# Audio-WestlakeU/FN-SSL

Hardware: AMD Instinct MI355X
Metric: TF-frames/sec DP-IPD forward, 4-mic 257-bin x 300-frame (higher is better)
Workload: dtype f32; 1 GPU; BASELINE configs[1]: FN-SSL (online) DP-IPD forward, waveform->STFT->features->3x(full-band BiLSTM + narrow-band LSTM)->head; 32 utterances/GPU x 4 mics ('MM' = 6 pairs) x 257 bins x 300 frames, fp32; frame = one STFT frame of one utterance; stream_chunk_frames=0, utterances_per_gpu=32, global_batch=32, mics=4, pairs_per_utterance=6, frames=300, bins=257, parallelism=dp1 (utterance shards, no collective), chunk_pairs=0

## Files before the change

fn-ssl_amd/csrc/lstm_f32c.h:

```cpp
#pragma once

#include "lstm_static.h"

namespace fnssl_lstm {

constexpr int kF32cWaves = 16;

struct F32ClusterParams {
  unsigned* tags;
  unsigned* status;
  int clusters_per_dir;
  int groups_per_cluster;
  unsigned spin_limit;
  int stall_member;
  int rotate;
  int prio_mode;
};

template <int HH, int NV0, int NS0, int MODE, bool ABLRT = false, int DRIFT = 2, int NW_ = kF32cWaves, int GS = 1>
__global__ void __launch_bounds__(NW_ * 64) lstm_f32c_kernel(const LstmParams p, const F32ClusterParams cp) {
  constexpr int H = HH, NS = H / 16, NW = NW_;
  constexpr int NWS = NW / GS;
  static_assert((GS == 1 || GS == 4) && NW % GS == 0 && (NWS & (NWS - 1)) == 0, "gate split: whole slots, a power of two of them");
  constexpr bool SUM = (MODE & kSum) != 0, SAVE = (MODE & kSave) != 0;
  constexpr bool CAT = (MODE & kHas2) != 0;
  constexpr int QPS = 1 + NV0 + NS0 + NS;
  constexpr int XD = NW_ > 12 ? 4 : 8;
  constexpr bool STRH = H == 256 && GS == 1 && NW_ > 8;
  static_assert((CAT ? NS0 == 1 : !(NV0 && NS0)) && (NV0 == 0 || NV0 % XD == 0) && (H == 128 || H == 256),
                "blocks of src0, or its remainder alone, or blocks of src0 + the remainder quad of src2");
  static_assert(H == 128 || NW_ <= 8 || STRH, "H = 256 with the row of h_{t-1} held: at most two waves per SIMD (register budget)");
  static_assert(!STRH || (NV0 >= XD && (NV0 + NS) % XD == 0), "streamed row: the ring depth divides the block count");
  static_assert(GS == 1 || (!SAVE && !ABLRT), "gate split: inference kernels only");
  extern __shared__ __attribute__((aligned(16))) char smem[];
  const int ABL = ABLRT ? p.ablate : 0;

  const int b = blockIdx.x;
  const int m = (b >> 3) % NS;
  const int cl = ((b >> 3) / NS) * 8 + (b & 7);
  if (cl >= cp.clusters_per_dir * p.ndir) return;
  const int dir = cl / cp.clusters_per_dir;
  const int ck = cl - dir * cp.clusters_per_dir;
  const int g0 = ck * cp.groups_per_cluster;
  const int g1 = g0 + cp.groups_per_cluster < p.ntasks ? g0 + cp.groups_per_cluster : p.ntasks;
  if (__hip_atomic_load(cp.status, __ATOMIC_RELAXED, __HIP_MEMORY_SCOPE_AGENT) != 0) return;
  if (cl == 0 && m == cp.stall_member) return;

  const int lane = threadIdx.x & 63;
  const int n = lane & 15, g = lane >> 4;
  const int w = __builtin_amdgcn_readfirstlane((int)(threadIdx.x >> 6));
  const int ws = GS == 1 ? w : (w >> 2);
  const int gate = GS == 1 ? 0 : (w & 3);
  const bool rev = dir == 1;
  const unsigned vlane = lane * 16;

  {
    const v4f* src = reinterpret_cast<const v4f*>(reinterpret_cast<const char*>(p.wpack[dir]) + (size_t)(m * QPS) * 4096);
    v4f* dst = reinterpret_cast<v4f*>(smem);
    for (int i = threadIdx.x; i < QPS * 4 * 64; i += NW * 64) dst[i] = src[i];
  }
  char* const xch = smem + QPS * 4096;
  unsigned* const xcnt = reinterpret_cast<unsigned*>(xch + NWS * 2 * 4 * 1024);
  if (GS > 1 && threadIdx.x < NWS) xcnt[threadIdx.x] = 0;
  __syncthreads();
  const char* const lds_rd = smem + lane * 16;
  auto rec = [&](int q, int j) { return *reinterpret_cast<const v4f*>(lds_rd + (q * 4 + j) * 1024); };
  auto rec1 = [&](int q, int j) { return *reinterpret_cast<const float*>(lds_rd + (q * 4 + j) * 1024 + 4 * gate); };

  const unsigned st0 = (unsigned)(p.src0.st * 4), sto = (unsigned)(p.out_st * 4), stk = SUM ? (unsigned)(p.skip.st * 4) : 0u;
  const unsigned st2 = CAT ? (unsigned)(p.src2.st * 4) : 0u;
  const unsigned cy = (unsigned)p.carry;
  unsigned* const tag_cl = cp.tags + (size_t)cl * cp.groups_per_cluster * NS;
  const v4f zero4 = v4f{0.f, 0.f, 0.f, 0.f};

  unsigned pub_val = 0;
  unsigned* pub_tag = nullptr;
  auto pub_flush = [&]() {
    if (pub_tag) {
      asm volatile("s_waitcnt vmcnt(0)" ::: "memory");
      if (lane == 0) __hip_atomic_store(pub_tag, pub_val, __ATOMIC_RELAXED, __HIP_MEMORY_SCOPE_AGENT);
      pub_tag = nullptr;
    }
  };

  struct Grp {
    unsigned vo0, voo, vok, voo2, vo2 = 0;
    bool valid;
    int task, step;
  };
  auto locate = [&](int task, int qo0, int qi0, Grp& gr, rsrc_t& rx0, rsrc_t& ro, rsrc_t& rsk, rsrc_t& ro2, rsrc_t& rx2) {
    const int q0 = task * 16;
    gr.valid = q0 + n < p.nseq;
    const int d = q0 + n < p.nseq ? n : p.nseq - 1 - q0;
    const bool crossed = qi0 + d >= p.q_inner;
    auto one = [&](const float* base, long long so, long long si, int extra, unsigned& voff) {
      const long long delta = (long long)d * si + (crossed ? so - (long long)p.q_inner * si : 0ll);
      voff = (unsigned)(delta * 4) + (unsigned)(extra * 4);
      return make_rsrc(base + ((long long)qo0 * so + (long long)qi0 * si));
    };
    rx0 = one(p.src0.p, p.src0.so, p.src0.si, (NS0 && !CAT) ? g : 4 * g, gr.vo0);
    if constexpr (CAT) rx2 = one(p.src2.p, p.src2.so, p.src2.si, g, gr.vo2);
    ro = one(p.out, p.out_so, p.out_si, dir * H + 4 * g, gr.voo);
    gr.vok = gr.voo2 = 0;
    rsk = SUM ? one(p.skip.p, p.skip.so, p.skip.si, dir * H + 4 * g, gr.vok) : rx0;
    ro2 = SUM ? one(p.out_sum, p.out_so, p.out_si, dir * H + 4 * g, gr.voo2) : ro;
  };
  auto tt_of = [&](int step) { return (unsigned)(rev ? p.nsteps - 1 - step : step); };
  auto rc_of = [&](int task) {
    return make_rsrc(cell_record<NS>(p.cscratch, p.ntasks, dir, task));
  };

  if (g0 + ws >= g1) return;
  unsigned long long clk0 = 0, rt0 = 0;
  if (ABLRT && (ABL & 512)) {
    clk0 = __builtin_amdgcn_s_memtime();
    rt0 = __builtin_amdgcn_s_memrealtime();
  }
  bool dead = false;
  auto bounded_wait = [&](auto ready, auto reload, int sleep, unsigned code) {
    for (unsigned spins = 0; !ready(); ++spins) {
      if (GS > 1) __builtin_amdgcn_s_sleep(1); else if (sleep == 8) __builtin_amdgcn_s_sleep(8); else __builtin_amdgcn_s_sleep(16);
      reload();
      const bool out = spins > cp.spin_limit;
      if (out || (spins & 63) == 63) {
        if (out) {
          if (lane == 0) __hip_atomic_store(cp.status, code | (unsigned)(cl & 0xffff), __ATOMIC_RELAXED, __HIP_MEMORY_SCOPE_AGENT);
          return false;
        }
        if (__hip_atomic_load(cp.status, __ATOMIC_RELAXED, __HIP_MEMORY_SCOPE_AGENT) != 0) return false;
      }
    }
    return true;
  };
  const int NGR = g1 - g0;
  const bool rot = cp.rotate && NGR >= 2 * NWS;
  const int FULL = rot ? (NGR / NWS) * NWS : NGR, LEFT = NGR - FULL;
  const bool single = GS == 1 && g0 + ws + NWS >= g1;
  Grp cur, nxt;
  rsrc_t rx0, ro, rsk, ro2, rx2, nrx0, nro, nrsk, nro2, nrx2;
  v4f xr[XD];
  float xs0 = 0.f;
  v4f cprev = zero4, skipv = zero4;
  unsigned tagv = 0, tagd = 0;
  auto request = [&](const Grp& gr, rsrc_t qx0, rsrc_t qsk, bool with_c, bool with_x = true) {
    const unsigned tt = tt_of(gr.step);
    if (!(ABL & 8)) {
      if constexpr (NV0 > 0) if (with_x) static_for<XD>([&](auto v) { xr[v.value] = bld4(qx0, gr.vo0, tt * st0 + 64 * v.value); });
      if constexpr (NS0 > 0 && !CAT) xs0 = bld1(qx0, gr.vo0, tt * st0);
    }
    if (SUM && !(ABL & 64)) skipv = bld4(qsk, gr.vok, tt * stk + 64 * m);
    if (gr.step > 0 || cy) {
      if (gr.step > 0 && !(ABL & 256))
        tagv = __hip_atomic_load(tag_cl + (size_t)(gr.task - g0) * NS + (lane & (NS - 1)), __ATOMIC_RELAXED, __HIP_MEMORY_SCOPE_AGENT);
      if (GS == 1 && with_c && !(ABL & 64)) cprev = bld4_l2(rc_of(gr.task), vlane, m * 1024);
    }
    if (DRIFT > 0 && !(ABL & 256) && gr.task - DRIFT * NWS >= g0)
      tagd = __hip_atomic_load(tag_cl + (size_t)(gr.task - DRIFT * NWS - g0) * NS + (lane & (NS - 1)), __ATOMIC_RELAXED, __HIP_MEMORY_SCOPE_AGENT);
  };
  cur.task = g0 + ws;
  cur.step = 0;
  unsigned iter = 0;
  const int qo_first = (cur.task * 16) / p.q_inner, qi_first = cur.task * 16 - qo_first * p.q_inner;
  int qo0 = qo_first, qi0 = qi_first;
  locate(cur.task, qo0, qi0, cur, rx0, ro, rsk, ro2, rx2);
  request(cur, rx0, rsk, true);
  if constexpr (CAT) xs0 = bld1(rx2, cur.vo2, tt_of(0) * st2);

  for (;;) {
    const int step = cur.step, task = cur.task;
    const unsigned tt = tt_of(step);
    const unsigned o0 = tt * st0, oo = (tt + cy) * sto;
    const unsigned op = (rev ? tt + 1 : tt - 1 + cy) * sto;
    const rsrc_t rc = rc_of(task);
    unsigned* const tag_g = tag_cl + (size_t)(task - g0) * NS;
    if (single && (step > 0 || cy) && !(ABL & 64)) cprev = bld4_l2(rc, vlane, m * 1024);
    const bool late_c = GS > 1 || task >= g0 + FULL;
    v4f cprev_cur = (step > 0 || cy) ? cprev : zero4;
    const v4f skip_cur = skipv;

    v4f hold[STRH ? 1 : NS];
    auto fetch_h = [&]() {
      if (DRIFT > 0 && !(ABL & 4) && !dead && task - DRIFT * NWS >= g0) {
        unsigned* const tag_d = tag_cl + (size_t)(task - DRIFT * NWS - g0) * NS;
        dead = !bounded_wait([&]() { return __builtin_amdgcn_ballot_w64(tagd < (unsigned)step + 1) == 0; },
                             [&]() { tagd = __hip_atomic_load(tag_d + (lane & (NS - 1)), __ATOMIC_RELAXED, __HIP_MEMORY_SCOPE_AGENT); }, 8, 0x40000u);
      }
      if ((step > 0 || cy) && !(ABL & 16)) {
        if (step > 0 && !(ABL & 4) && !dead)
          dead = !bounded_wait([&]() { return __builtin_amdgcn_ballot_w64(tagv < (unsigned)step) == 0; },
                               [&]() { tagv = __hip_atomic_load(tag_g + (lane & (NS - 1)), __ATOMIC_RELAXED, __HIP_MEMORY_SCOPE_AGENT); }, 16, 0x30000u);
        if (late_c && !(ABL & 64)) cprev_cur = bld4_l2(rc, vlane, m * 1024);
        if constexpr (!STRH) {
#pragma unroll
          for (int s = 0; s < NS; ++s) hold[s] = bld4_l2(ro, cur.voo, op + 64 * s);
        }
      } else if constexpr (!STRH) {
#pragma unroll
        for (int s = 0; s < NS; ++s) hold[s] = (ABL & 16) ? cprev : zero4;
      }
    };
    const bool hrow = step > 0 || cy;
    auto hblock = [&](int j) { return hrow ? bld4_l2(ro, cur.voo, op + 64 * j) : zero4; };

    if (cp.prio_mode == 2) __builtin_amdgcn_s_setprio(2);
    v4f acc[4];
    v4f ra[4];
    v4f acc1 = zero4;
    float rb[4] = {0.f, 0.f, 0.f, 0.f};
    if constexpr (GS == 1) {
      acc[0] = rec(0, 0);
      acc[1] = rec(0, 1);
      acc[2] = rec(0, 2);
      acc[3] = rec(0, 3);
      static_for<4>([&](auto j) { ra[j.value] = rec(1, j.value); });
    } else {
      acc1 = rec(0, gate);
      static_for<4>([&](auto j) { rb[j.value] = rec1(1, j.value); });
    }
    auto quad = [&](auto qc, float b0, float b1, float b2, float b3) {
      constexpr int Q = decltype(qc)::value;
      if constexpr (GS > 1) {
        acc1 = __builtin_amdgcn_mfma_f32_16x16x4f32(rb[0], b0, acc1, 0, 0, 0);
        if constexpr (Q + 1 < QPS) rb[0] = rec1(Q + 1, 0);
        acc1 = __builtin_amdgcn_mfma_f32_16x16x4f32(rb[1], b1, acc1, 0, 0, 0);
        if constexpr (Q + 1 < QPS) rb[1] = rec1(Q + 1, 1);
        acc1 = __builtin_amdgcn_mfma_f32_16x16x4f32(rb[2], b2, acc1, 0, 0, 0);
        if constexpr (Q + 1 < QPS) rb[2] = rec1(Q + 1, 2);
        acc1 = __builtin_amdgcn_mfma_f32_16x16x4f32(rb[3], b3, acc1, 0, 0, 0);
        if constexpr (Q + 1 < QPS) rb[3] = rec1(Q + 1, 3);
        return;
      }
      MFMA4(acc, ra[0], b0);
      __builtin_amdgcn_sched_barrier(0);
      if constexpr (Q + 1 < QPS) if (!(ABL & 128)) ra[0] = rec(Q + 1, 0);
      __builtin_amdgcn_sched_barrier(0);
// ... 3 lines not shown
      __builtin_amdgcn_sched_barrier(0);
      MFMA4(acc, ra[2], b2);
      __builtin_amdgcn_sched_barrier(0);
      if constexpr (Q + 1 < QPS) if (!(ABL & 128)) ra[2] = rec(Q + 1, 2);
      __builtin_amdgcn_sched_barrier(0);
      MFMA4(acc, ra[3], b3);
      __builtin_amdgcn_sched_barrier(0);
      if constexpr (Q + 1 < QPS) if (!(ABL & 128)) ra[3] = rec(Q + 1, 3);
      __builtin_amdgcn_sched_barrier(0);
    };
    auto quad1 = [&](auto qc, float b0) {
      constexpr int Q = decltype(qc)::value;
      if constexpr (GS > 1) {
        acc1 = __builtin_amdgcn_mfma_f32_16x16x4f32(rb[0], b0, acc1, 0, 0, 0);
        if constexpr (Q + 1 < QPS) static_for<4>([&](auto j) { rb[j.value] = rec1(Q + 1, j.value); });
        return;
      }
      MFMA4(acc, ra[0], b0);
      if constexpr (Q + 1 < QPS) static_for<4>([&](auto j) { ra[j.value] = rec(Q + 1, j.value); });
    };
    if constexpr (NV0 > 0) {
      static_for<NV0>([&](auto v) {
        constexpr int V = decltype(v)::value;
        if constexpr (STRH) {
          if constexpr (V == NV0 / 2) pub_flush();
          if constexpr (V == NV0 - XD) fetch_h();
        } else if constexpr (V == NV0 / 2) {
          pub_flush();
          fetch_h();
        }
        const v4f xb = xr[V % XD];
        quad(ic<1 + V>{}, xb.x, xb.y, xb.z, xb.w);
        if constexpr (V + XD < NV0) {
          if (!(ABL & 8)) xr[V % XD] = bld4(rx0, cur.vo0, o0 + 64 * (V + XD));
        } else if constexpr (STRH) {
          xr[V % XD] = hblock(V + XD - NV0);
        }
      });
      if constexpr (NS0 > 0) quad1(ic<1 + NV0>{}, xs0);
    } else {
      pub_flush();
      fetch_h();
      quad1(ic<1>{}, xs0);
    }
    bool seq_next = false;
    if (task < g0 + FULL && task + NWS < g0 + FULL) {
      nxt.task = task + NWS;
      nxt.step = step;
      seq_next = true;
    } else {
      const int j = (ws - step) & (NWS - 1);
      if (task < g0 + FULL && j < LEFT) {
        nxt.task = g0 + FULL + j;
        nxt.step = step;
      } else {
        nxt.task = g0 + ws;
        nxt.step = step + 1;
      }
    }
    const bool more = nxt.step < p.nsteps;
    if (more) {
      if (ABL & 1) {
        nxt.vo0 = cur.vo0; nxt.voo = cur.voo; nxt.vok = cur.vok; nxt.voo2 = cur.voo2; nxt.valid = cur.valid;
        nrx0 = rx0; nro = ro; nrsk = rsk; nro2 = ro2;
        if constexpr (CAT) {
          nxt.vo2 = cur.vo2;
          nrx2 = rx2;
        }
      } else {
        if (seq_next) {
          qi0 += 16 * NWS;
          while (qi0 >= p.q_inner) {
            qi0 -= p.q_inner;
            ++qo0;
          }
        } else if (nxt.step == step) {
          qo0 = (nxt.task * 16) / p.q_inner;
          qi0 = nxt.task * 16 - qo0 * p.q_inner;
        } else {
          qo0 = qo_first;
          qi0 = qi_first;
        }
        locate(nxt.task, qo0, qi0, nxt, nrx0, nro, nrsk, nro2, nrx2);
      }
      request(nxt, nrx0, nrsk, !single && nxt.task < g0 + FULL, !STRH);
      if constexpr (CAT) xs0 = bld1(nrx2, nxt.vo2, tt_of(nxt.step) * st2);
    }
    static_for<NS>([&](auto sp) {
      constexpr int SP = decltype(sp)::value;
      if constexpr (STRH) {
        constexpr int B = NV0 + SP, B2 = B + XD;
        const v4f hb = xr[B % XD];
        quad(ic<1 + NV0 + NS0 + SP>{}, hb.x, hb.y, hb.z, hb.w);
        if constexpr (B2 < NV0 + NS) {
          xr[B % XD] = hblock(B2 - NV0);
        } else {
          if (more) xr[B % XD] = bld4(nrx0, nxt.vo0, tt_of(nxt.step) * st0 + 64 * (B2 - NV0 - NS));
        }
      } else {
        quad(ic<1 + NV0 + NS0 + SP>{}, hold[SP].x, hold[SP].y, hold[SP].z, hold[SP].w);
      }
    });

    if (cp.prio_mode == 2) __builtin_amdgcn_s_setprio(0);
    if (dead) break;
    v4f cn, hn;
    if (ABL & 2) {
      cn = acc[1] + cprev_cur + acc[0];
      hn = acc[3] + acc[2];
    } else {
      v4f ig, fg, gg, og;
      if constexpr (GS == 1) {
        ig = sigmoid4(acc[0]);
        fg = sigmoid4(acc[1]);
        gg = tanh4(acc[2]);
        og = sigmoid4(acc[3]);
      } else {
        const v4f act = gate == 2 ? tanh4(acc1) : sigmoid4(acc1);
        v4f* const xb = reinterpret_cast<v4f*>(xch + (size_t)((ws * 2 + (int)(iter & 1u)) * 4) * 1024);
        xb[gate * 64 + lane] = act;
        asm volatile("s_waitcnt lgkmcnt(0)" ::: "memory");
        if (lane == 0) __hip_atomic_fetch_add(xcnt + ws, 1u, __ATOMIC_RELAXED, __HIP_MEMORY_SCOPE_WORKGROUP);
        const unsigned want = 4u * (iter + 1u);
        for (unsigned spins = 0;; ++spins) {
          if (__hip_atomic_load(xcnt + ws, __ATOMIC_RELAXED, __HIP_MEMORY_SCOPE_WORKGROUP) >= want) break;
          if (dead || ((spins & 63u) == 63u && __hip_atomic_load(cp.status, __ATOMIC_RELAXED, __HIP_MEMORY_SCOPE_AGENT) != 0u) ||
              spins > cp.spin_limit) {
            dead = true;
            break;
          }
          __builtin_amdgcn_s_sleep(1);
        }
        asm volatile("" ::: "memory");
        ig = xb[lane];
        fg = xb[64 + lane];
        gg = xb[128 + lane];
        og = xb[192 + lane];
        ++iter;
      }
      cn = cell4(fg, cprev_cur, ig, gg);
      hn = mul_rn4(og, tanh4(cn));
      if constexpr (SAVE) {
        const rsrc_t rres = make_rsrc(reinterpret_cast<const char*>(p.reserve) +
                                      ((size_t)dir * p.ntasks + task) * p.nsteps * (size_t)(NS * kReserveRecs * 1024));
        const unsigned rb = (tt * NS + m) * (kReserveRecs * 1024);
        bst4(ig, rres, vlane, rb);
        bst4(fg, rres, vlane, rb + 1024);
        bst4(gg, rres, vlane, rb + 2048);
        bst4(og, rres, vlane, rb + 3072);
        bst4(cn, rres, vlane, rb + 4096);
      }
    }
    asm("" : "+v"(hn.x), "+v"(hn.y), "+v"(hn.z), "+v"(hn.w));
    if (ABL & 32) asm volatile("" ::"v"(cn), "v"(hn));
    const bool storer = GS == 1 || gate == 0;
    if (storer && !(ABL & 32)) bst4(cn, rc, vlane, m * 1024);
    if (storer && cur.valid && !(ABL & 32)) {
      __builtin_amdgcn_raw_buffer_store_b128(__builtin_bit_cast(v4u, hn), ro, cur.voo, oo + 64 * m, 16);
      if (SUM) bst4(add_rn4(hn, skip_cur), ro2, cur.voo2, oo + 64 * m);
    }
    pub_val = __builtin_amdgcn_readfirstlane((unsigned)step + 1);
    pub_tag = ((ABL & 256) || !storer) ? nullptr : tag_g + m;
    if (GS > 1 || single) pub_flush();
    if (!more || dead) break;
    cur = nxt;
    rx0 = nrx0;
    ro = nro;
    rsk = nrsk;
    ro2 = nro2;
    if constexpr (CAT) rx2 = nrx2;
  }
  pub_flush();
  asm volatile("s_waitcnt vmcnt(0)" ::: "memory");
  if (ABLRT && (ABL & 512) && (w == 0 || w == 15) && lane == 0) {
    const unsigned long long c1 = __builtin_amdgcn_s_memtime(), r1 = __builtin_amdgcn_s_memrealtime();
    printf("f32c blk %d wave %d start %llu end %llu cycles %llu MHz %.1f\n", b, w, rt0, r1, c1 - clk0,
           (double)(c1 - clk0) / (double)(r1 - rt0) * 100.0);
  }
}

template <int HH, int NV0, int NS0, int MODE, bool ABLRT = false, int DRIFT = 2, int NW_ = kF32cWaves, int GS = 1>
int launch_f32c_k(const LstmParams& p, const F32ClusterParams& cp, const LaunchCtx& lc) {
  constexpr int NS = HH / 16;
  constexpr int QPS = 1 + NV0 + NS0 + NS;
  const size_t lds = (size_t)QPS * 4096 + (GS > 1 ? (size_t)(NW_ / GS) * 8192 + 64 : 0);
  static_assert(QPS * 4096 + (GS > 1 ? (NW_ / GS) * 8192 + 64 : 0) <= 160 * 1024, "LDS");
  const int ncl = cp.clusters_per_dir * p.ndir;
  const int nwg = 8 * NS * ((ncl + 7) / 8);
  return enqueue(lc, Kernel{lstm_f32c_kernel<HH, NV0, NS0, MODE, ABLRT, DRIFT, NW_, GS>, NW_ * 64, lds, "lstm_f32c_kernel", true}, nwg, p, cp);
}

}
```

fn-ssl_amd/csrc/lstm_f32c.hip:

```cpp
#include <cstdlib>

#include "lstm_f32c.h"
#include "tuning.h"

namespace fnssl_lstm {

constexpr int kF32cWavesH256 = 16;
constexpr int kF32cWavesH256Split = 8;

static bool f32c_uniform(const LstmParams& p, int mode) {
  auto even = [&](long long so, long long si) { return si >= 0 && so == (long long)p.q_inner * si; };
  return even(p.src0.so, p.src0.si) && even(p.out_so, p.out_si) && (!(mode & kSum) || even(p.skip.so, p.skip.si)) &&
         (!(mode & kHas2) || even(p.src2.so, p.src2.si));
}

bool f32c_handles(const LstmParams& p, int H, int mode) {
  if (fnssl::tune(FNSSL_TUNE_NO_F32_CLUSTER)) return false;
  if ((H != 128 && H != 256) || p.ablate) return false;
  if (H == 128) {
    if (p.c2 != 0 || p.carry) return false;
    if (p.reserve && mode != 0) return false;
    if (!(p.c0 == 256 && (mode == kSum || mode == 0)) && !(p.c0 == 4 && mode == 0 && !fnssl::tune(FNSSL_TUNE_NO_F32C_B1))) return false;
  } else {
    if (p.ndir != 1 || p.c0 != 256 || fnssl::tune(FNSSL_TUNE_NO_F32_SMALL)) return false;
    const bool plain = p.c2 == 0 && (mode == 0 || mode == kSum), cat = p.c2 == 4 && (mode == kHas2 || mode == (kHas2 | kSum));
    if (!plain && !cat) return false;
    if (p.reserve && ((mode & kSum) || p.carry)) return false;
  }
  auto grows = [&](long long so, long long si) { return si >= 0 && so >= (long long)(p.q_inner - 1) * si; };
  if (!f32c_uniform(p, mode) &&
      (p.q_inner < 16 || !grows(p.src0.so, p.src0.si) || !grows(p.out_so, p.out_si) ||
       ((mode & kSum) && !grows(p.skip.so, p.skip.si)) || ((mode & kHas2) && !grows(p.src2.so, p.src2.si))))
    return false;
  const int ncu = cluster_cus();
  if (ncu < (H / 16) * p.ndir) return false;
  const long long groups = (long long)p.ntasks * p.ndir;
  if (const int mg = fnssl::tune(FNSSL_TUNE_F32C_MIN_GROUPS, 1, 1 << 30)) {
    if (groups < mg) return false;
  }
  if (p.reserve) {
    if (fnssl::tune(FNSSL_TUNE_TRAIN_NO_F32_CLUSTER)) return false;
    return true;
  }
  if (H == 256) {
    const long long full = 12LL * ncu, rounds = (groups + full - 1) / full;
    return groups < full || groups * 100 < rounds * full * 97;
  }
  return !fnssl::tune(FNSSL_TUNE_NO_F32_SMALL) || groups >= 12LL * ncu;
}

template <int NW_, int GS>
static int launch_f32c_h256(const LstmParams& p, const F32ClusterParams& cp, int mode, const LaunchCtx& lc) {
  if (mode == (kHas2 | kSum)) return launch_f32c_k<256, 16, 1, kHas2 | kSum, false, 2, NW_, GS>(p, cp, lc);
  if (mode == kHas2) return launch_f32c_k<256, 16, 1, kHas2, false, 2, NW_, GS>(p, cp, lc);
  if (mode == kSum) return launch_f32c_k<256, 16, 0, kSum, false, 2, NW_, GS>(p, cp, lc);
  return launch_f32c_k<256, 16, 0, 0, false, 2, NW_, GS>(p, cp, lc);
}

int forward_f32c(LstmParams p, int H, int mode, size_t cluster_bytes, const LaunchCtx& lc) {
  if (f32c_uniform(p, mode)) p.q_inner = p.nseq;
  const int ncu = cluster_cus();
  const int members = H / 16;
  F32ClusterParams cp;
  cp.clusters_per_dir = (ncu / members) / p.ndir;
  cp.groups_per_cluster = (p.ntasks + cp.clusters_per_dir - 1) / cp.clusters_per_dir;
  cp.status = reinterpret_cast<unsigned*>(p.cluster_ws);
  cp.tags = reinterpret_cast<unsigned*>(p.cluster_ws + 256);
  cp.spin_limit = cluster_spin_limit();
  cp.stall_member = cluster_test_stall();
  cp.rotate = !fnssl::tune(FNSSL_TUNE_F32C_NO_ROTATE);
  cp.prio_mode = fnssl::tune(FNSSL_TUNE_F32C_PRIO, 9, 9) ? 0 : 2;
  const size_t tag_bytes = (size_t)p.ndir * cp.clusters_per_dir * cp.groups_per_cluster * members * sizeof(unsigned);
  FNSSL_REQUIRE(256 + tag_bytes <= cluster_bytes, "lstm_forward: the cluster kernel's tags exceed the workspace's cluster area");
  if (!lc.dry) FNSSL_HIP(hipMemsetAsync(p.cluster_ws, 0, 256 + tag_bytes, lc.st));
  const int gs_knob = fnssl::tune(FNSSL_TUNE_F32C_GATE_SPLIT, 1, 4);
  const bool gsplit = gs_knob ? gs_knob == 4 : cp.groups_per_cluster <= 1;
  if (H == 256) {
    constexpr int W = kF32cWavesH256;
    if (p.reserve)
      return p.c2 == 4 ? launch_f32c_k<256, 16, 1, kHas2 | kSave, false, 2, W>(p, cp, lc) : launch_f32c_k<256, 16, 0, kSave, false, 2, W>(p, cp, lc);
    if (gsplit) return launch_f32c_h256<kF32cWavesH256Split, 4>(p, cp, mode, lc);
    if (cp.groups_per_cluster <= kF32cWavesH256Split) return launch_f32c_h256<kF32cWavesH256Split, 1>(p, cp, mode, lc);
    return launch_f32c_h256<W, 1>(p, cp, mode, lc);
  }
  if (gsplit && !p.reserve) {
    if (p.c0 == 4) return launch_f32c_k<128, 0, 1, 0, false, 2, kF32cWaves, 4>(p, cp, lc);
    if (mode == kSum) return launch_f32c_k<128, 16, 0, kSum, false, 2, kF32cWaves, 4>(p, cp, lc);
    return launch_f32c_k<128, 16, 0, 0, false, 2, kF32cWaves, 4>(p, cp, lc);
  }
#ifdef FNSSL_BUILD_ABLATE
  if (const int abl = env_int("FNSSL_F32C_ABL", 1, 1023)) {
    p.ablate = abl;
    if (mode == kSum) return launch_f32c_k<128, 16, 0, kSum, true>(p, cp, lc);
    if (p.c0 == 4) return launch_f32c_k<128, 0, 1, 0, true>(p, cp, lc);
  }
  p.ablate = 0;
#endif
  if (p.reserve) return p.c0 == 4 ? launch_f32c_k<128, 0, 1, kSave>(p, cp, lc) : launch_f32c_k<128, 16, 0, kSave>(p, cp, lc);
  if (p.c0 == 4) return launch_f32c_k<128, 0, 1, 0>(p, cp, lc);
  if (mode == kSum) return launch_f32c_k<128, 16, 0, kSum>(p, cp, lc);
  return launch_f32c_k<128, 16, 0, 0>(p, cp, lc);
}

}
```

fn-ssl_amd/csrc/runtime.hip:

```cpp
#include <atomic>
#include <cstring>
#include <map>
#include <mutex>
#include <string>
#include <vector>

#include "common.h"
#include "tuning.h"
#include "lstm_host.h"

namespace fnssl {

int device_cus() {
  static std::mutex mu;
  static int cache[64] = {0};
  int dev = 0;
  if (hipGetDevice(&dev) != hipSuccess || dev < 0 || dev >= 64) return 256;
  std::lock_guard<std::mutex> lk(mu);
  if (cache[dev] == 0) {
    int n = 0;
    if (hipDeviceGetAttribute(&n, hipDeviceAttributeMultiprocessorCount, dev) != hipSuccess || n <= 0) n = 256;
    cache[dev] = n;
  }
  return cache[dev];
// ... 21 lines not shown
    "LSTM_CHQ",
    "NO_F32_CLUSTER",
    "NO_F32C_B1",
    "TRAIN_NO_F32_CLUSTER",
    "F32C_NO_ROTATE",
    "F32C_PRIO",
    "NO_CLUSTER",
    "NO_CLUSTER_B1",
    "NO_CLUSTER_H128",
    "CLUSTER_SPREAD",
    "BF16P_DRAIN",
    "BF16W_SOLO",
    "BWD_NO_CLUSTER",
    "BWD_CLUSTER_MIN_GROUPS",
    "BWD_CLUSTER_NO_ROTATE",
    "BWDC_NO_PREFETCH",
    "BWDC_NO_TOKEN",
    "BWDC_WAVES16",
    "FWD_RING",
    "BWD_RING",
    "TRAIN_SPLIT",
    "TRAIN_NO_STATIC",
    "NO_FWD2",
    "NO_BWD2",
    "SN_SCALAR",
    "STFT_PER_FRAME",
    "CLUSTER_SPIN_LIMIT",
    "CLUSTER_TEST_STALL",
    "RESERVED_CUS",
    "NO_F32_SMALL",
    "F32C_MIN_GROUPS",
    "F32C_GATE_SPLIT",
    "CLUSTER_FULL_TILES",
    "NO_STATIC4"};
constexpr int kTuneNamed = (int)(sizeof(kTuneNames) / sizeof(kTuneNames[0]));
static_assert(kTuneNamed <= FNSSL_TUNE_COUNT, "more knob names than slots");
static_assert(kTuneNamed == FNSSL_TUNE_NO_STATIC4 + 1, "knob names out of step with include/fnssl.h");
}

const fnssl_tuning& tuning() {
  if (g_call_tuning) return *g_call_tuning;
  const unsigned v = g_tuning_version.load(std::memory_order_acquire);
  if (v != g_thread_version) {
    std::lock_guard<std::mutex> lk(g_tuning_mu);
    g_thread_tuning = g_default_tuning;
    g_thread_version = g_tuning_version.load(std::memory_order_relaxed);
  }
  return g_thread_tuning;
}

TuningScope::TuningScope(const fnssl_tuning* t) : prev_(g_call_tuning), active_(false) {
  if (t && t->struct_bytes == sizeof(fnssl_tuning)) {
    g_call_tuning = t;
    active_ = true;
  }
}
TuningScope::~TuningScope() {
  if (active_) g_call_tuning = prev_;
}

void set_error(const char* fmt, ...) {
  va_list ap;
  va_start(ap, fmt);
  vsnprintf(g_err, sizeof(g_err), fmt, ap);
  va_end(ap);
}

namespace {
struct Rec {
  const char* name;
// ... 215 lines not shown
```

fn-ssl_amd/fnssl/_lib.py:

```python
from __future__ import annotations

import ctypes as C
import os

import torch

_HERE = os.path.dirname(os.path.abspath(__file__))
LIB_PATH = os.path.join(os.path.dirname(_HERE), "csrc", "libfnssl_hip.so")
LIB_PATH = os.environ.get("FNSSL_LIB_PATH", LIB_PATH)

ABI_VERSION = 19
CH_MODE = {"M": 0, "MM": 1}
STREAM_MODE = {"pair": 0, "array": 1}
LSTM_FAMILY = {1: "generic", 2: "static", 3: "static2 (retired)", 4: "split", 5: "split_static", 6: "f32_cluster",
               7: "static3", 8: "bf16", 9: "bf16_solo", 10: "bf16_pair", 11: "bf16_cluster", 12: "train", 13: "bwd", 14: "bwd_cluster",
               15: "static4"}

SYMBOLS = [
    "fnssl_abi_version", "fnssl_last_error", "fnssl_tuning_set", "fnssl_tuning_get", "fnssl_tuning_name", "fnssl_occupy_cus", "fnssl_num_frames", "fnssl_num_pairs", "fnssl_stft",
    "fnssl_num_frames_ex", "fnssl_stft_ex", "fnssl_array_frontend",
    "fnssl_forgetting_coefs", "fnssl_pair_features", "fnssl_nchw_to_seq", "fnssl_lstm_packed_floats",
    "fnssl_lstm_pack", "fnssl_lstm_workspace_bytes", "fnssl_lstm_workspace_bytes_ex", "fnssl_lstm_plan_rounds", "fnssl_lstm_plan", "fnssl_lstm_forward", "fnssl_lstm_cluster_status", "fnssl_head", "fnssl_linear",
    "fnssl_ipd2doa", "fnssl_doa_peaks", "fnssl_dpipd_targets", "fnssl_conv3x3_packed_floats", "fnssl_conv3x3_pack", "fnssl_conv3x3_causal",
    "fnssl_avgpool_time", "fnssl_array_features", "fnssl_conv3x3_packed_floats_bf16", "fnssl_conv3x3_pack_bf16",
# ... 350 lines not shown
    for name in ("fnssl_sn_fconv_backward_workspace_bytes", "fnssl_sn_full_backward_workspace_bytes"):
        getattr(lib, name).argtypes = [i, i, i]
        getattr(lib, name).restype = sz
    lib.fnssl_sn_fconv_backward.argtypes = [PV, i, i, i, C.POINTER(SnFconvW), i, i, vp, ll, ll, ll, vp, ll, ll, ll,
                                            C.POINTER(SnFconvGrads), vp, sz, vp]
    lib.fnssl_sn_full_backward.argtypes = [PV, i, i, i, C.POINTER(SnFullW), i, vp, ll, ll, ll, vp, ll, ll, ll,
                                           C.POINTER(SnFullGrads), vp, sz, vp]
    lib.fnssl_sn_head.argtypes = [PV, i, i, i, vp, vp, vp, vp, vp, vp]
    lib.fnssl_sn_encoder_backward_workspace_bytes.argtypes = [i, i, i, i]
    lib.fnssl_sn_encoder_backward_workspace_bytes.restype = sz
    lib.fnssl_sn_encoder_backward.argtypes = [vp, ll, ll, ll, ll, i, i, i, i, vp, vp, ll, ll, ll, vp, vp, vp, ll, ll, ll, ll,
                                              vp, sz, vp]
    lib.fnssl_sn_head_backward_workspace_bytes.argtypes = [i, i, i]
    lib.fnssl_sn_head_backward_workspace_bytes.restype = sz
    lib.fnssl_sn_head_backward.argtypes = [PV, i, i, i, vp, vp, vp, vp, vp, ll, ll, ll, C.POINTER(SnHeadGrads), vp, sz, vp]
    lib.fnssl_sn_forward_workspace_bytes.argtypes = [i, i, i]
    lib.fnssl_sn_forward_workspace_bytes.restype = sz
    lib.fnssl_sn_state_floats.argtypes = [C.POINTER(SnNet), i, i]
    lib.fnssl_sn_state_floats.restype = sz
    lib.fnssl_sn_forward.argtypes = [C.POINTER(SnNet), vp, ll, ll, ll, ll, i, i, i, vp, i, vp, vp, sz, vp]
    lib.fnssl_sn_state_rows.argtypes = [C.POINTER(SnNet), i, i, vp, i, vp, C.POINTER(C.c_int), C.POINTER(C.c_ubyte), i, vp]
    lib.fnssl_timing_enable.argtypes = [i]
    lib.fnssl_timing_select.argtypes = [C.c_char_p]
    lib.fnssl_timing_collect.argtypes = [i, vp, vp, vp, vp]
    if lib.fnssl_abi_version() != ABI_VERSION:
        raise RuntimeError("fnssl: ABI version mismatch (library %d, binding %d)"
                           % (lib.fnssl_abi_version(), ABI_VERSION))
    _lib = lib
    refresh_tuning()
    return lib


_tune_index = None
_PRESENCE = {"NO_F32_CLUSTER", "NO_F32C_B1", "TRAIN_NO_F32_CLUSTER", "F32C_NO_ROTATE", "NO_CLUSTER", "NO_CLUSTER_B1",
             "NO_CLUSTER_H128", "CLUSTER_SPREAD", "BF16W_SOLO", "SN_SCALAR", "STFT_PER_FRAME"}
_ENV_ALIAS = {"LSTM_NO_STATIC": "FNSSL_LSTM_NO_STATIC"}


def tuning_names():
    global _tune_index
    if _tune_index is None:
        lib = _lib
        if lib is None:
            raise RuntimeError("fnssl: load() first")
        idx, k = {}, 0
        while True:
            n = lib.fnssl_tuning_name(k)
            if n is None:
                break
            idx[n.decode()] = k
            k += 1
        _tune_index = idx
    return _tune_index


def tuning_from_env(environ=None) -> Tuning:
    environ = os.environ if environ is None else environ
    t = Tuning()
    t.struct_bytes = C.sizeof(Tuning)
    for name, k in tuning_names().items():
        v = environ.get(_ENV_ALIAS.get(name, "FNSSL_" + name))
        if v is None:
            continue
        try:
            iv = int(v)
        except ValueError:
            iv = 1
# ... 55 lines not shown
```

include/fnssl.h:

```cpp
#ifndef FNSSL_H_
#define FNSSL_H_

#include <stddef.h>

#ifdef __cplusplus
extern "C" {
#endif

#define FNSSL_ABI_VERSION 19

#define FNSSL_OK 0
#define FNSSL_E_INVALID (-1)
#define FNSSL_E_HIP (-2)
#define FNSSL_E_WORKSPACE (-3)

#define FNSSL_CH_MODE_M 0
#define FNSSL_CH_MODE_MM 1

#define FNSSL_WIN_LEN 512
#define FNSSL_HOP 256
#define FNSSL_NBIN 257
#define FNSSL_NF 256
#define FNSSL_SEG_FRAMES 12

// ... 13 lines not shown
#define FNSSL_TUNE_NO_F32_CLUSTER 9
#define FNSSL_TUNE_NO_F32C_B1 10
#define FNSSL_TUNE_TRAIN_NO_F32_CLUSTER 11
#define FNSSL_TUNE_F32C_NO_ROTATE 12
#define FNSSL_TUNE_F32C_PRIO 13
#define FNSSL_TUNE_NO_CLUSTER 14
#define FNSSL_TUNE_NO_CLUSTER_B1 15
#define FNSSL_TUNE_NO_CLUSTER_H128 16
#define FNSSL_TUNE_CLUSTER_SPREAD 17
#define FNSSL_TUNE_BF16P_DRAIN 18
#define FNSSL_TUNE_BF16W_SOLO 19
#define FNSSL_TUNE_BWD_NO_CLUSTER 20
#define FNSSL_TUNE_BWD_CLUSTER_MIN_GROUPS 21
#define FNSSL_TUNE_BWD_CLUSTER_NO_ROTATE 22
#define FNSSL_TUNE_BWDC_NO_PREFETCH 23
#define FNSSL_TUNE_BWDC_NO_TOKEN 24
#define FNSSL_TUNE_BWDC_WAVES16 25
#define FNSSL_TUNE_FWD_RING 26
#define FNSSL_TUNE_BWD_RING 27
#define FNSSL_TUNE_TRAIN_SPLIT 28
#define FNSSL_TUNE_TRAIN_NO_STATIC 29
#define FNSSL_TUNE_NO_FWD2 30
#define FNSSL_TUNE_NO_BWD2 31
#define FNSSL_TUNE_SN_SCALAR 32
#define FNSSL_TUNE_STFT_PER_FRAME 33
#define FNSSL_TUNE_CLUSTER_SPIN_LIMIT 34
#define FNSSL_TUNE_CLUSTER_TEST_STALL 35
#define FNSSL_TUNE_RESERVED_CUS 36
#define FNSSL_TUNE_NO_F32_SMALL 37
#define FNSSL_TUNE_F32C_MIN_GROUPS 38
#define FNSSL_TUNE_F32C_GATE_SPLIT 39
#define FNSSL_TUNE_CLUSTER_FULL_TILES 40
#define FNSSL_TUNE_NO_STATIC4 41
#define FNSSL_TUNE_COUNT 48

typedef struct fnssl_tuning {
  unsigned struct_bytes;
  int knob[FNSSL_TUNE_COUNT];
} fnssl_tuning;

int fnssl_tuning_set(const fnssl_tuning* t);
int fnssl_tuning_get(fnssl_tuning* t);
const char* fnssl_tuning_name(int index);

int fnssl_occupy_cus(int nblocks, int lds_bytes, unsigned* stop, int max_ms, void* stream);


int fnssl_num_frames(int ns);

int fnssl_num_pairs(int nch, int ch_mode);

int fnssl_stft(const float* sig, int nb, int ns, int nch,
               long long sb, long long sn, long long sc,
               float* spec, float* magsum, void* stream);

int fnssl_num_frames_ex(int ns, int hop, int center);
int fnssl_stft_ex(const float* sig, int nb, int ns, int nch,
                  long long sb, long long sn, long long sc, int hop, int center,
                  float* spec, float* magsum, void* stream);

int fnssl_forgetting_coefs(int nt, int sample_length, float* a, float* b);

int fnssl_pair_features(const float* spec, const float* magsum,
                        const float* coef_a, const float* coef_b,
                        int nb, int nch, int nt, int ch_mode, float eps,
                        float* mu, float* x, int layout, void* stream);
// ... 529 lines not shown
```

Measured before the change: 17120 frames/s.

## Map f32 cluster LSTM task groups onto 2-D sequence tiles for H=128

Adds a tiled mapping for the H=128 f32 cluster LSTM kernel. Each 16-sequence task group becomes an a-by-b tile over the outer/inner sequence axes rather than 16 consecutive sequences, so per-lane offsets are fixed and only a scalar group offset changes between groups. Cell state is addressed per cluster base, and buffer resources are built once. This aims to cut per-group address recomputation and resource rebuilding, and lets strided layouts that previously fell back use the cluster kernel. The cost is more template instances, a new eligibility check, and 32-bit offset limits that the check must respect.

Result: no change. 17180 frames/s (median of 5 runs) (+0.4%).

```diff
diff --git a/fn-ssl_amd/csrc/lstm_f32c.h b/fn-ssl_amd/csrc/lstm_f32c.h
--- a/fn-ssl_amd/csrc/lstm_f32c.h
+++ b/fn-ssl_amd/csrc/lstm_f32c.h
@@ -1,5 +1,6 @@
 #pragma once
 
+#include "lstm_group_tile.h"
 #include "lstm_static.h"
 
 namespace fnssl_lstm {
@@ -17,7 +18,7 @@
   int prio_mode;
 };
 
-template <int HH, int NV0, int NS0, int MODE, bool ABLRT = false, int DRIFT = 2, int NW_ = kF32cWaves, int GS = 1>
+template <int HH, int NV0, int NS0, int MODE, bool ABLRT = false, int DRIFT = 2, int NW_ = kF32cWaves, int GS = 1, bool TILED = false>
 __global__ void __launch_bounds__(NW_ * 64) lstm_f32c_kernel(const LstmParams p, const F32ClusterParams cp) {
   constexpr int H = HH, NS = H / 16, NW = NW_;
   constexpr int NWS = NW / GS;
@@ -32,6 +33,7 @@
   static_assert(H == 128 || NW_ <= 8 || STRH, "H = 256 with the row of h_{t-1} held: at most two waves per SIMD (register budget)");
   static_assert(!STRH || (NV0 >= XD && (NV0 + NS) % XD == 0), "streamed row: the ring depth divides the block count");
   static_assert(GS == 1 || (!SAVE && !ABLRT), "gate split: inference kernels only");
+  static_assert(!TILED || (H == 128 && !SAVE && !CAT && !ABLRT && (!SUM || NV0 > 0)), "tiled groups: the H = 128 inference kernels");
   extern __shared__ __attribute__((aligned(16))) char smem[];
   const int ABL = ABLRT ? p.ablate : 0;
 
@@ -85,10 +87,31 @@
 
   struct Grp {
     unsigned vo0, voo, vok, voo2, vo2 = 0;
+    unsigned s0 = 0, so = 0;
     bool valid;
     int task, step;
   };
+  const GroupTile gt = group_tile(p.q_inner);
+  int qo_base = 0, qi_base = 0;
+  if constexpr (TILED) tile_of_task(g0 + ws, p.q_inner, gt, qo_base, qi_base);
+  const unsigned so4x = tile_stride32(p.src0.so), si4x = tile_stride32(p.src0.si), so4o = tile_stride32(p.out_so), si4o = tile_stride32(p.out_si);
+  const unsigned tvo0 = TILED ? tile_lane_offset32(n, gt, so4x, si4x) + (unsigned)(((NS0 && !CAT) ? g : 4 * g) * 4) : 0u;
+  const unsigned tvoo = TILED ? tile_lane_offset32(n, gt, so4o, si4o) + (unsigned)(4 * g * 4) : 0u;
+  const unsigned sdir = (unsigned)(dir * H * 4);
+  auto V0 = [&](const Grp& gr) { if constexpr (TILED) return tvo0; else return gr.vo0; };
+  auto VO = [&](const Grp& gr) { if constexpr (TILED) return tvoo; else return gr.voo; };
+  auto VK = [&](const Grp& gr) { if constexpr (TILED) return tvo0; else return gr.vok; };
+  auto VO2 = [&](const Grp& gr) { if constexpr (TILED) return tvoo; else return gr.voo2; };
+  auto S0 = [&](const Grp& gr) { if constexpr (TILED) return gr.s0; else return 0u; };
+  auto SO = [&](const Grp& gr) { if constexpr (TILED) return gr.so; else return 0u; };
+  auto SK = [&](const Grp& gr) { if constexpr (TILED) return gr.s0 + sdir; else return 0u; };
   auto locate = [&](int task, int qo0, int qi0, Grp& gr, rsrc_t& rx0, rsrc_t& ro, rsrc_t& rsk, rsrc_t& ro2, rsrc_t& rx2) {
+    if constexpr (TILED) {
+      gr.s0 = tile_group_offset32(qo0, qi0, qo_base, so4x, si4x);
+      gr.so = tile_group_offset32(qo0, qi0, qo_base, so4o, si4o) + sdir;
+      gr.valid = true;
+      return;
+    }
     const int q0 = task * 16;
     gr.valid = q0 + n < p.nseq;
     const int d = q0 + n < p.nseq ? n : p.nseq - 1 - q0;
@@ -107,8 +130,9 @@
   };
   auto tt_of = [&](int step) { return (unsigned)(rev ? p.nsteps - 1 - step : step); };
   auto rc_of = [&](int task) {
-    return make_rsrc(cell_record<NS>(p.cscratch, p.ntasks, dir, task));
-  };
+    return make_rsrc(cell_record<NS>(p.cscratch, p.ntasks, dir, TILED ? g0 : task));
+  };
+  auto cs_of = [&](int task) { return (TILED ? (unsigned)(task - g0) * (unsigned)(NS * 1024) : 0u) + (unsigned)(m * 1024); };
 
   if (g0 + ws >= g1) return;
   unsigned long long clk0 = 0, rt0 = 0;
@@ -145,14 +169,14 @@
   auto request = [&](const Grp& gr, rsrc_t qx0, rsrc_t qsk, bool with_c, bool with_x = true) {
     const unsigned tt = tt_of(gr.step);
     if (!(ABL & 8)) {
-      if constexpr (NV0 > 0) if (with_x) static_for<XD>([&](auto v) { xr[v.value] = bld4(qx0, gr.vo0, tt * st0 + 64 * v.value); });
-      if constexpr (NS0 > 0 && !CAT) xs0 = bld1(qx0, gr.vo0, tt * st0);
-    }
-    if (SUM && !(ABL & 64)) skipv = bld4(qsk, gr.vok, tt * stk + 64 * m);
+      if constexpr (NV0 > 0) if (with_x) static_for<XD>([&](auto v) { xr[v.value] = bld4(qx0, V0(gr), S0(gr) + tt * st0 + 64 * v.value); });
+      if constexpr (NS0 > 0 && !CAT) xs0 = bld1(qx0, V0(gr), S0(gr) + tt * st0);
+    }
+    if (SUM && !(ABL & 64)) skipv = bld4(qsk, VK(gr), SK(gr) + tt * stk + 64 * m);
     if (gr.step > 0 || cy) {
       if (gr.step > 0 && !(ABL & 256))
         tagv = __hip_atomic_load(tag_cl + (size_t)(gr.task - g0) * NS + (lane & (NS - 1)), __ATOMIC_RELAXED, __HIP_MEMORY_SCOPE_AGENT);
-      if (GS == 1 && with_c && !(ABL & 64)) cprev = bld4_l2(rc_of(gr.task), vlane, m * 1024);
+      if (GS == 1 && with_c && !(ABL & 64)) cprev = bld4_l2(rc_of(gr.task), vlane, cs_of(gr.task));
     }
     if (DRIFT > 0 && !(ABL & 256) && gr.task - DRIFT * NWS >= g0)
       tagd = __hip_atomic_load(tag_cl + (size_t)(gr.task - DRIFT * NWS - g0) * NS + (lane & (NS - 1)), __ATOMIC_RELAXED, __HIP_MEMORY_SCOPE_AGENT);
@@ -160,7 +184,16 @@
   cur.task = g0 + ws;
   cur.step = 0;
   unsigned iter = 0;
-  const int qo_first = (cur.task * 16) / p.q_inner, qi_first = cur.task * 16 - qo_first * p.q_inner;
+  int qo_first = (cur.task * 16) / p.q_inner, qi_first = cur.task * 16 - qo_first * p.q_inner;
+  if constexpr (TILED) {
+    qo_first = qo_base;
+    qi_first = qi_base;
+    const long long base = (long long)qo_base;
+    rx0 = nrx0 = make_rsrc(p.src0.p + base * p.src0.so);
+    ro = nro = make_rsrc(p.out + base * p.out_so);
+    rsk = nrsk = SUM ? make_rsrc(p.skip.p + base * p.skip.so) : rx0;
+    ro2 = nro2 = SUM ? make_rsrc(p.out_sum + base * p.out_so) : ro;
+  }
   int qo0 = qo_first, qi0 = qi_first;
   locate(cur.task, qo0, qi0, cur, rx0, ro, rsk, ro2, rx2);
   request(cur, rx0, rsk, true);
@@ -169,11 +202,11 @@
   for (;;) {
     const int step = cur.step, task = cur.task;
     const unsigned tt = tt_of(step);
-    const unsigned o0 = tt * st0, oo = (tt + cy) * sto;
-    const unsigned op = (rev ? tt + 1 : tt - 1 + cy) * sto;
+    const unsigned o0 = S0(cur) + tt * st0, oo = SO(cur) + (tt + cy) * sto;
+    const unsigned op = SO(cur) + (rev ? tt + 1 : tt - 1 + cy) * sto;
     const rsrc_t rc = rc_of(task);
     unsigned* const tag_g = tag_cl + (size_t)(task - g0) * NS;
-    if (single && (step > 0 || cy) && !(ABL & 64)) cprev = bld4_l2(rc, vlane, m * 1024);
+    if (single && (step > 0 || cy) && !(ABL & 64)) cprev = bld4_l2(rc, vlane, cs_of(task));
     const bool late_c = GS > 1 || task >= g0 + FULL;
     v4f cprev_cur = (step > 0 || cy) ? cprev : zero4;
     const v4f skip_cur = skipv;
@@ -189,10 +222,10 @@
         if (step > 0 && !(ABL & 4) && !dead)
           dead = !bounded_wait([&]() { return __builtin_amdgcn_ballot_w64(tagv < (unsigned)step) == 0; },
                                [&]() { tagv = __hip_atomic_load(tag_g + (lane & (NS - 1)), __ATOMIC_RELAXED, __HIP_MEMORY_SCOPE_AGENT); }, 16, 0x30000u);
-        if (late_c && !(ABL & 64)) cprev_cur = bld4_l2(rc, vlane, m * 1024);
+        if (late_c && !(ABL & 64)) cprev_cur = bld4_l2(rc, vlane, cs_of(task));
         if constexpr (!STRH) {
 #pragma unroll
-          for (int s = 0; s < NS; ++s) hold[s] = bld4_l2(ro, cur.voo, op + 64 * s);
+          for (int s = 0; s < NS; ++s) hold[s] = bld4_l2(ro, VO(cur), op + 64 * s);
         }
       } else if constexpr (!STRH) {
 #pragma unroll
@@ -200,7 +233,7 @@
       }
     };
     const bool hrow = step > 0 || cy;
-    auto hblock = [&](int j) { return hrow ? bld4_l2(ro, cur.voo, op + 64 * j) : zero4; };
+    auto hblock = [&](int j) { return hrow ? bld4_l2(ro, VO(cur), op + 64 * j) : zero4; };
 
     if (cp.prio_mode == 2) __builtin_amdgcn_s_setprio(2);
     v4f acc[4];
@@ -270,7 +303,7 @@
         const v4f xb = xr[V % XD];
         quad(ic<1 + V>{}, xb.x, xb.y, xb.z, xb.w);
         if constexpr (V + XD < NV0) {
-          if (!(ABL & 8)) xr[V % XD] = bld4(rx0, cur.vo0, o0 + 64 * (V + XD));
+          if (!(ABL & 8)) xr[V % XD] = bld4(rx0, V0(cur), o0 + 64 * (V + XD));
         } else if constexpr (STRH) {
           xr[V % XD] = hblock(V + XD - NV0);
         }
@@ -300,6 +333,7 @@
     if (more) {
       if (ABL & 1) {
         nxt.vo0 = cur.vo0; nxt.voo = cur.voo; nxt.vok = cur.vok; nxt.voo2 = cur.voo2; nxt.valid = cur.valid;
+        nxt.s0 = cur.s0; nxt.so = cur.so;
         nrx0 = rx0; nro = ro; nrsk = rsk; nro2 = ro2;
         if constexpr (CAT) {
           nxt.vo2 = cur.vo2;
@@ -307,14 +341,18 @@
         }
       } else {
         if (seq_next) {
-          qi0 += 16 * NWS;
+          qi0 += (TILED ? gt.b : 16) * NWS;
           while (qi0 >= p.q_inner) {
             qi0 -= p.q_inner;
-            ++qo0;
+            qo0 += TILED ? gt.a : 1;
           }
         } else if (nxt.step == step) {
-          qo0 = (nxt.task * 16) / p.q_inner;
-          qi0 = nxt.task * 16 - qo0 * p.q_inner;
+          if constexpr (TILED) {
+            tile_of_task(nxt.task, p.q_inner, gt, qo0, qi0);
+          } else {
+            qo0 = (nxt.task * 16) / p.q_inner;
+            qi0 = nxt.task * 16 - qo0 * p.q_inner;
+          }
         } else {
           qo0 = qo_first;
           qi0 = qi_first;
@@ -333,7 +371,7 @@
         if constexpr (B2 < NV0 + NS) {
           xr[B % XD] = hblock(B2 - NV0);
         } else {
-          if (more) xr[B % XD] = bld4(nrx0, nxt.vo0, tt_of(nxt.step) * st0 + 64 * (B2 - NV0 - NS));
+          if (more) xr[B % XD] = bld4(nrx0, V0(nxt), S0(nxt) + tt_of(nxt.step) * st0 + 64 * (B2 - NV0 - NS));
         }
       } else {
         quad(ic<1 + NV0 + NS0 + SP>{}, hold[SP].x, hold[SP].y, hold[SP].z, hold[SP].w);
@@ -392,20 +430,22 @@
     asm("" : "+v"(hn.x), "+v"(hn.y), "+v"(hn.z), "+v"(hn.w));
     if (ABL & 32) asm volatile("" ::"v"(cn), "v"(hn));
     const bool storer = GS == 1 || gate == 0;
-    if (storer && !(ABL & 32)) bst4(cn, rc, vlane, m * 1024);
-    if (storer && cur.valid && !(ABL & 32)) {
-      __builtin_amdgcn_raw_buffer_store_b128(__builtin_bit_cast(v4u, hn), ro, cur.voo, oo + 64 * m, 16);
-      if (SUM) bst4(add_rn4(hn, skip_cur), ro2, cur.voo2, oo + 64 * m);
+    if (storer && !(ABL & 32)) bst4(cn, rc, vlane, cs_of(task));
+    if (storer && (TILED || cur.valid) && !(ABL & 32)) {
+      __builtin_amdgcn_raw_buffer_store_b128(__builtin_bit_cast(v4u, hn), ro, VO(cur), oo + 64 * m, 16);
+      if (SUM) bst4(add_rn4(hn, skip_cur), ro2, VO2(cur), oo + 64 * m);
     }
     pub_val = __builtin_amdgcn_readfirstlane((unsigned)step + 1);
     pub_tag = ((ABL & 256) || !storer) ? nullptr : tag_g + m;
     if (GS > 1 || single) pub_flush();
     if (!more || dead) break;
     cur = nxt;
-    rx0 = nrx0;
-    ro = nro;
-    rsk = nrsk;
-    ro2 = nro2;
+    if constexpr (!TILED) {
+      rx0 = nrx0;
+      ro = nro;
+      rsk = nrsk;
+      ro2 = nro2;
+    }
     if constexpr (CAT) rx2 = nrx2;
   }
   pub_flush();
@@ -417,7 +457,7 @@
   }
 }
 
-template <int HH, int NV0, int NS0, int MODE, bool ABLRT = false, int DRIFT = 2, int NW_ = kF32cWaves, int GS = 1>
+template <int HH, int NV0, int NS0, int MODE, bool ABLRT = false, int DRIFT = 2, int NW_ = kF32cWaves, int GS = 1, bool TILED = false>
 int launch_f32c_k(const LstmParams& p, const F32ClusterParams& cp, const LaunchCtx& lc) {
   constexpr int NS = HH / 16;
   constexpr int QPS = 1 + NV0 + NS0 + NS;
@@ -425,7 +465,7 @@
   static_assert(QPS * 4096 + (GS > 1 ? (NW_ / GS) * 8192 + 64 : 0) <= 160 * 1024, "LDS");
   const int ncl = cp.clusters_per_dir * p.ndir;
   const int nwg = 8 * NS * ((ncl + 7) / 8);
-  return enqueue(lc, Kernel{lstm_f32c_kernel<HH, NV0, NS0, MODE, ABLRT, DRIFT, NW_, GS>, NW_ * 64, lds, "lstm_f32c_kernel", true}, nwg, p, cp);
+  return enqueue(lc, Kernel{lstm_f32c_kernel<HH, NV0, NS0, MODE, ABLRT, DRIFT, NW_, GS, TILED>, NW_ * 64, lds, "lstm_f32c_kernel", true}, nwg, p, cp);
 }
 
 }
diff --git a/fn-ssl_amd/csrc/lstm_f32c.hip b/fn-ssl_amd/csrc/lstm_f32c.hip
--- a/fn-ssl_amd/csrc/lstm_f32c.hip
+++ b/fn-ssl_amd/csrc/lstm_f32c.hip
@@ -14,6 +14,27 @@
          (!(mode & kHas2) || even(p.src2.so, p.src2.si));
 }
 
+static bool f32c_tiled(LstmParams& p, int H, int mode) {
+  if (H != 128 || p.reserve || p.carry || p.c2 != 0 || (mode & ~kSum) || fnssl::tune(FNSSL_TUNE_F32C_NO_TILE)) return false;
+  const int clusters_per_dir = (cluster_cus() / (H / 16)) / p.ndir;
+  if (clusters_per_dir < 1) return false;
+  const int groups_per_cluster = (p.ntasks + clusters_per_dir - 1) / clusters_per_dir;
+  LstmParams r = p;
+  if (f32c_uniform(p, mode)) {
+    r.q_inner = 16;
+    r.src0.so = 16 * p.src0.si;
+    r.out_so = 16 * p.out_si;
+    r.skip.so = 16 * p.skip.si;
+  }
+  const TileTensor v[3] = {{r.src0.so, r.src0.si, r.src0.st, r.c0},
+                           {r.out_so, r.out_si, r.out_st, 2 * H},
+                           {r.skip.so, r.skip.si, r.skip.st, 2 * H}};
+  if ((mode & kSum) && (r.skip.so != r.src0.so || r.skip.si != r.src0.si)) return false;
+  if (!tile_mapping_ok(r.nseq, r.q_inner, groups_per_cluster, r.nsteps, v, (mode & kSum) ? 3 : 2)) return false;
+  p = r;
+  return true;
+}
+
 bool f32c_handles(const LstmParams& p, int H, int mode) {
   if (fnssl::tune(FNSSL_TUNE_NO_F32_CLUSTER)) return false;
   if ((H != 128 && H != 256) || p.ablate) return false;
@@ -28,7 +49,8 @@
     if (p.reserve && ((mode & kSum) || p.carry)) return false;
   }
   auto grows = [&](long long so, long long si) { return si >= 0 && so >= (long long)(p.q_inner - 1) * si; };
-  if (!f32c_uniform(p, mode) &&
+  LstmParams as_tiles = p;
+  if (!f32c_uniform(p, mode) && !f32c_tiled(as_tiles, H, mode) &&
       (p.q_inner < 16 || !grows(p.src0.so, p.src0.si) || !grows(p.out_so, p.out_si) ||
        ((mode & kSum) && !grows(p.skip.so, p.skip.si)) || ((mode & kHas2) && !grows(p.src2.so, p.src2.si))))
     return false;
@@ -57,8 +79,16 @@
   return launch_f32c_k<256, 16, 0, 0, false, 2, NW_, GS>(p, cp, lc);
 }
 
+template <int GS, bool TILED>
+static int launch_f32c_h128(const LstmParams& p, const F32ClusterParams& cp, int mode, const LaunchCtx& lc) {
+  if (p.c0 == 4) return launch_f32c_k<128, 0, 1, 0, false, 2, kF32cWaves, GS, TILED>(p, cp, lc);
+  if (mode == kSum) return launch_f32c_k<128, 16, 0, kSum, false, 2, kF32cWaves, GS, TILED>(p, cp, lc);
+  return launch_f32c_k<128, 16, 0, 0, false, 2, kF32cWaves, GS, TILED>(p, cp, lc);
+}
+
 int forward_f32c(LstmParams p, int H, int mode, size_t cluster_bytes, const LaunchCtx& lc) {
-  if (f32c_uniform(p, mode)) p.q_inner = p.nseq;
+  bool tiled = f32c_tiled(p, H, mode);
+  if (!tiled && f32c_uniform(p, mode)) p.q_inner = p.nseq;
   const int ncu = cluster_cus();
   const int members = H / 16;
   F32ClusterParams cp;
@@ -83,23 +113,18 @@
     if (cp.groups_per_cluster <= kF32cWavesH256Split) return launch_f32c_h256<kF32cWavesH256Split, 1>(p, cp, mode, lc);
     return launch_f32c_h256<W, 1>(p, cp, mode, lc);
   }
-  if (gsplit && !p.reserve) {
-    if (p.c0 == 4) return launch_f32c_k<128, 0, 1, 0, false, 2, kF32cWaves, 4>(p, cp, lc);
-    if (mode == kSum) return launch_f32c_k<128, 16, 0, kSum, false, 2, kF32cWaves, 4>(p, cp, lc);
-    return launch_f32c_k<128, 16, 0, 0, false, 2, kF32cWaves, 4>(p, cp, lc);
-  }
+  if (gsplit && !p.reserve) return tiled ? launch_f32c_h128<4, true>(p, cp, mode, lc) : launch_f32c_h128<4, false>(p, cp, mode, lc);
 #ifdef FNSSL_BUILD_ABLATE
   if (const int abl = env_int("FNSSL_F32C_ABL", 1, 1023)) {
     p.ablate = abl;
+    tiled = false;
     if (mode == kSum) return launch_f32c_k<128, 16, 0, kSum, true>(p, cp, lc);
     if (p.c0 == 4) return launch_f32c_k<128, 0, 1, 0, true>(p, cp, lc);
   }
   p.ablate = 0;
 #endif
   if (p.reserve) return p.c0 == 4 ? launch_f32c_k<128, 0, 1, kSave>(p, cp, lc) : launch_f32c_k<128, 16, 0, kSave>(p, cp, lc);
-  if (p.c0 == 4) return launch_f32c_k<128, 0, 1, 0>(p, cp, lc);
-  if (mode == kSum) return launch_f32c_k<128, 16, 0, kSum>(p, cp, lc);
-  return launch_f32c_k<128, 16, 0, 0>(p, cp, lc);
+  return tiled ? launch_f32c_h128<1, true>(p, cp, mode, lc) : launch_f32c_h128<1, false>(p, cp, mode, lc);
 }
 
 }
diff --git a/fn-ssl_amd/csrc/lstm_group_tile.h b/fn-ssl_amd/csrc/lstm_group_tile.h
--- /dev/null
+++ b/fn-ssl_amd/csrc/lstm_group_tile.h
@@ -0,0 +1,81 @@
+#pragma once
+
+#if defined(__HIPCC__) || defined(__CUDACC__)
+#define FNSSL_TILE_HD __host__ __device__ inline __attribute__((always_inline))
+#else
+#define FNSSL_TILE_HD inline
+#endif
+
+namespace fnssl_lstm {
+
+struct GroupTile {
+  int a, b;
+  int lb;
+};
+
+FNSSL_TILE_HD GroupTile group_tile(int q_inner) {
+  const int low = q_inner & -q_inner;
+  const int b = low < 16 ? low : 16;
+  const int lb = __builtin_ctz((unsigned)b);
+  return GroupTile{16 >> lb, b, lb};
+}
+
+FNSSL_TILE_HD int tile_tasks_inner(int q_inner, GroupTile t) { return q_inner >> t.lb; }
+
+FNSSL_TILE_HD void tile_of_task(int task, int q_inner, GroupTile t, int& qo0, int& qi0) {
+  const int tin = tile_tasks_inner(q_inner, t);
+  const int ot = task / tin;
+  qo0 = ot * t.a;
+  qi0 = (task - ot * tin) * t.b;
+}
+
+FNSSL_TILE_HD void tile_lane(int n, GroupTile t, int& qo, int& qi) {
+  qi = n & (t.b - 1);
+  qo = n >> t.lb;
+}
+
+FNSSL_TILE_HD unsigned tile_stride32(long long s) { return (unsigned)((unsigned long long)s * 4ull); }
+
+FNSSL_TILE_HD unsigned tile_lane_offset32(int n, GroupTile t, unsigned so4, unsigned si4) {
+  int qo, qi;
+  tile_lane(n, t, qo, qi);
+  return (unsigned)qo * so4 + (unsigned)qi * si4;
+}
+
+FNSSL_TILE_HD unsigned tile_group_offset32(int qo0, int qi0, int qo_base, unsigned so4, unsigned si4) {
+  return (unsigned)(qo0 - qo_base) * so4 + (unsigned)qi0 * si4;
+}
+
+struct TileTensor {
+  long long so, si, st;
+  long long width;
+};
+
+inline int tile_cluster_span(int ntasks, int groups_per_cluster, int tasks_inner) {
+  int span = 0;
+  for (int g0 = 0; g0 < ntasks; g0 += groups_per_cluster) {
+    const int g1 = g0 + groups_per_cluster < ntasks ? g0 + groups_per_cluster : ntasks;
+    const int s = (g1 - 1) / tasks_inner - g0 / tasks_inner + 1;
+    span = s > span ? s : span;
+  }
+  return span;
+}
+
+inline long double tile_extent_bytes(const TileTensor& v, int q_inner, int nsteps, GroupTile t, int span) {
+  return (((long double)span * t.a - 1.0L) * (long double)v.so + (long double)(q_inner - 1) * (long double)v.si +
+          (long double)nsteps * (long double)v.st + (long double)v.width) * 4.0L;
+}
+
+inline bool tile_mapping_ok(int nseq, int q_inner, int groups_per_cluster, int nsteps, const TileTensor* v, int nv) {
+  if (nseq <= 0 || q_inner <= 0 || groups_per_cluster <= 0 || nsteps <= 0 || nseq % q_inner != 0) return false;
+  const GroupTile t = group_tile(q_inner);
+  if ((nseq / q_inner) % t.a != 0) return false;
+  const int span = tile_cluster_span(nseq / 16, groups_per_cluster, tile_tasks_inner(q_inner, t));
+  for (int i = 0; i < nv; ++i) {
+    if (v[i].so < 0 || v[i].si < 0 || v[i].st < 0 || v[i].width < 0) return false;
+    if (!(tile_extent_bytes(v[i], q_inner, nsteps, t, span) < 4.0e9L)) return false;
+  }
+  return true;
+}
+
+}
diff --git a/fn-ssl_amd/csrc/runtime.hip b/fn-ssl_amd/csrc/runtime.hip
--- a/fn-ssl_amd/csrc/runtime.hip
+++ b/fn-ssl_amd/csrc/runtime.hip
@@ -77,10 +77,11 @@
     "F32C_MIN_GROUPS",
     "F32C_GATE_SPLIT",
     "CLUSTER_FULL_TILES",
-    "NO_STATIC4"};
+    "NO_STATIC4",
+    "F32C_NO_TILE"};
 constexpr int kTuneNamed = (int)(sizeof(kTuneNames) / sizeof(kTuneNames[0]));
 static_assert(kTuneNamed <= FNSSL_TUNE_COUNT, "more knob names than slots");
-static_assert(kTuneNamed == FNSSL_TUNE_NO_STATIC4 + 1, "knob names out of step with include/fnssl.h");
+static_assert(kTuneNamed == FNSSL_TUNE_F32C_NO_TILE + 1, "knob names out of step with include/fnssl.h");
 }
 
 const fnssl_tuning& tuning() {
diff --git a/fn-ssl_amd/fnssl/_lib.py b/fn-ssl_amd/fnssl/_lib.py
--- a/fn-ssl_amd/fnssl/_lib.py
+++ b/fn-ssl_amd/fnssl/_lib.py
@@ -406,7 +406,7 @@
 
 
 _tune_index = None
-_PRESENCE = {"NO_F32_CLUSTER", "NO_F32C_B1", "TRAIN_NO_F32_CLUSTER", "F32C_NO_ROTATE", "NO_CLUSTER", "NO_CLUSTER_B1",
+_PRESENCE = {"NO_F32_CLUSTER", "NO_F32C_B1", "TRAIN_NO_F32_CLUSTER", "F32C_NO_ROTATE", "F32C_NO_TILE", "NO_CLUSTER", "NO_CLUSTER_B1",
              "NO_CLUSTER_H128", "CLUSTER_SPREAD", "BF16W_SOLO", "SN_SCALAR", "STFT_PER_FRAME"}
 _ENV_ALIAS = {"LSTM_NO_STATIC": "FNSSL_LSTM_NO_STATIC"}
 
diff --git a/include/fnssl.h b/include/fnssl.h
--- a/include/fnssl.h
+++ b/include/fnssl.h
@@ -69,6 +69,7 @@
 #define FNSSL_TUNE_F32C_GATE_SPLIT 39
 #define FNSSL_TUNE_CLUSTER_FULL_TILES 40
 #define FNSSL_TUNE_NO_STATIC4 41
+#define FNSSL_TUNE_F32C_NO_TILE 42
 #define FNSSL_TUNE_COUNT 48
 
 typedef struct fnssl_tuning {
```
